# alibaba/unified-audio

Hardware: NVIDIA B200
Metric: hcodec2_encode_rvq_decode_samples_per_s (higher is better)
Workload: dtype f16x3/f16 tensor-core, f32 accumulate

## Files before the change

### unified_audio_b200/csrc/lstm_tc.cu

```cuda
#include <atomic>
#include <cstdio>
#include <cstdlib>

#include "common.cuh"
#include "quark_b200.h"

namespace qb {
extern std::atomic<long long> g_launches;

constexpr int LT_EPI_WARPS = 8, LT_THREADS = (LT_EPI_WARPS + 2) * 32;
constexpr int LT_KG = 4;
constexpr int LT_STAGES = 4;
constexpr uint32_t LT_KBLK = 32 * 128;
constexpr uint32_t LT_SLOT = LT_KBLK * LT_KG;
constexpr uint32_t LT_PAD = 12 * 1024;

__device__ __forceinline__ unsigned lt_ld_relaxed(const unsigned* p) {
  unsigned v;
  asm volatile("ld.relaxed.gpu.global.u32 %0, [%1];" : "=r"(v) : "l"(p) : "memory");
  return v;
}
__device__ __forceinline__ void bulk_load_1d(void* smem_dst, const void* gsrc, uint32_t bytes, uint64_t* bar) {
  asm volatile("cp.async.bulk.shared::cluster.global.mbarrier::complete_tx::bytes [%0], [%1], %2, [%3];"
               ::"r"(smem_u32(smem_dst)), "l"(gsrc), "r"(bytes), "r"(smem_u32(bar)) : "memory");
}
__device__ __forceinline__ void tmem_ld_32x32b_x8(uint32_t taddr, uint32_t (&r)[8]) {
  asm volatile("tcgen05.ld.sync.aligned.32x32b.x8.b32 {%0,%1,%2,%3,%4,%5,%6,%7}, [%8];"
               : "=r"(r[0]), "=r"(r[1]), "=r"(r[2]), "=r"(r[3]), "=r"(r[4]), "=r"(r[5]), "=r"(r[6]), "=r"(r[7])
               : "r"(taddr) : "memory");
}

__device__ __forceinline__ float lt_rcp(float x) {
  float r;
  asm("rcp.approx.ftz.f32 %0, %1;" : "=f"(r) : "f"(x));
  return r;
}
__device__ __forceinline__ float lt_sigmoid(float x) { return lt_rcp(1.0f + __expf(-x)); }
__device__ __forceinline__ float lt_tanh(float x) { return fmaf(-2.0f, lt_rcp(1.0f + __expf(2.0f * x)), 1.0f); }

__device__ __forceinline__ uint64_t lt_desc_core(uint32_t addr) {
  uint64_t d = 0;
  d |= (uint64_t)((addr & 0x3FFFF) >> 4);
  d |= (uint64_t)(128 >> 4) << 16;
  d |= (uint64_t)(128 >> 4) << 32;
  d |= (uint64_t)1 << 46;
  return d;
}
__device__ __forceinline__ void lt_cp_32x128b_warpx4(uint32_t taddr, uint64_t sdesc) {
  asm volatile("tcgen05.cp.cta_group::1.32x128b.warpx4 [%0], %1;" ::"r"(taddr), "l"(sdesc) : "memory");
}
__device__ __forceinline__ void lt_umma_ts(uint32_t tmem_d, uint32_t tmem_a, uint64_t desc_b, uint32_t idesc, uint32_t acc) {
  asm volatile(
      "{\n\t.reg .pred p;\n\t"
      "setp.ne.b32 p, %4, 0;\n\t"
      "tcgen05.mma.cta_group::1.kind::f16 [%0], [%1], %2, %3, p;\n\t}\n"
      ::"r"(tmem_d), "r"(tmem_a), "l"(desc_b), "r"(idesc), "r"(acc)
      : "memory");
}
constexpr uint32_t LT_TS_ACOL = 256;

template <int U, bool TS>
__global__ void __launch_bounds__(LT_THREADS, 1)
lstm_tc_kernel(const __grid_constant__ CUtensorMap tmW,
               const float* __restrict__ xp, int B, int T, int H, __half* __restrict__ out_hi,
               __half* __restrict__ out_lo, __half* hbuf, unsigned* flags, int Bp, int n_groups, int poll_ns, long long* prof) {
  constexpr int N = 4 * U;
  constexpr int HALF = U / 2;
  static_assert(N % 16 == 0 && N <= 64 && HALF * 4 % 8 == 0, "unsupported slice width");
  constexpr uint32_t WBLK = N * 128;
  constexpr uint32_t TCOLS = TS ? 512 : (4 * N <= 64 ? 64 : (4 * N <= 128 ? 128 : 256));
  extern __shared__ uint8_t smem_raw[];
  uint8_t* smem = (uint8_t*)(((uintptr_t)smem_raw + 1023) & ~(uintptr_t)1023);
  const int KB = H / 64;
  uint8_t* Wsm = smem;
  uint8_t* ring = smem + (size_t)KB * WBLK;
  uint64_t* full = (uint64_t*)(ring + LT_STAGES * LT_SLOT + LT_PAD);
  uint64_t* empty = full + LT_STAGES;
  uint64_t* wbar = empty + LT_STAGES;
  uint64_t* tfull = wbar + 1;
  uint32_t* tmem_slot = (uint32_t*)(tfull + 4);
  __shared__ long long ts_flag[4], ts_first[4], ts_last[4];

  const int tid = threadIdx.x, warp = tid >> 5, lane = tid & 31;
  const int u0 = blockIdx.x * U, G = gridDim.x;

  if (tid == 0) {
    for (int s = 0; s < LT_STAGES; ++s) { mbar_init(&full[s], 1); mbar_init(&empty[s], 1); }
    mbar_init(wbar, 1);
    for (int g = 0; g < 4; ++g) mbar_init(&tfull[g], 1);
    fence_mbar_init();
  }
  for (int i = tid; i < (int)((LT_STAGES * LT_SLOT + LT_PAD) / 16); i += LT_THREADS)
    reinterpret_cast<uint4*>(ring)[i] = make_uint4(0, 0, 0, 0);
  fence_proxy_async();
  if (warp == LT_EPI_WARPS + 1) { tmem_alloc(tmem_slot, TCOLS); tmem_relinquish(); }
  tc_fence_before();
  __syncthreads();
  tc_fence_after();
  const uint32_t tmem_base = *tmem_slot;

  if (warp == LT_EPI_WARPS) {
    if (lane == 0) {
      prefetch_tmap(&tmW);
      mbar_arrive_expect_tx(wbar, (uint32_t)KB * WBLK);
      for (int kb = 0; kb < KB; ++kb) tma_load_2d(Wsm + (size_t)kb * WBLK, &tmW, wbar, kb * 64, blockIdx.x * N);
    }
    uint32_t stage = 0, phase = 0;
    long long pw = 0;
    for (int t = 1; t < T; ++t) {
      for (int g = 0; g < n_groups; ++g) {
        const long long c0 = clock64();
        const unsigned* fl = flags + (size_t)g * G;
        unsigned spins = 0;
        for (;;) {
          bool ok = true;
          for (int c = lane; c < G; c += 32) ok = ok && (lt_ld_relaxed(fl + c) >= (unsigned)t);
          if (__all_sync(0xffffffffu, ok)) break;
          if (poll_ns) __nanosleep(poll_ns);
          if (++spins > (1u << 24)) asm volatile("trap;");
        }
        asm volatile("fence.acq_rel.gpu;" ::: "memory");
        __syncwarp();
        pw += clock64() - c0;
        if (lane == 0) {
          ts_flag[g] = clock64();
          asm volatile("fence.proxy.async;" ::: "memory");
          const int buf = (t + 1) & 1;
          for (int kb = 0; kb < KB; kb += LT_KG) {
            mbar_wait(&empty[stage], phase ^ 1);
            mbar_arrive_expect_tx(&full[stage], LT_SLOT);
            bulk_load_1d(ring + stage * LT_SLOT, hbuf + (((size_t)buf * n_groups + g) * KB + kb) * (LT_KBLK / 2), LT_SLOT,
                         &full[stage]);
            if (++stage == LT_STAGES) { stage = 0; phase ^= 1; }
          }
        }
        __syncwarp();
      }
    }
    if (prof && lane == 0 && blockIdx.x == 0) prof[0] = pw;
  } else if (warp == LT_EPI_WARPS + 1) {
    if (lane == 0) {
      constexpr uint32_t idesc = make_idesc_f16(128, N);
      mbar_wait(wbar, 0);
      uint32_t stage = 0, phase = 0, abuf = 0;
      for (int t = 1; t < T; ++t) {
        for (int g = 0; g < n_groups; ++g) {
          const uint32_t d_tmem = tmem_base + g * N;
          for (int kb0 = 0; kb0 < KB; kb0 += LT_KG) {
            mbar_wait(&full[stage], phase);
            tc_fence_after();
            if (kb0 == 0) ts_first[g] = clock64();
            if (TS) {
              const uint32_t a_tmem = tmem_base + LT_TS_ACOL + abuf * (LT_KG * 32);
              const uint32_t slot = smem_u32(ring + stage * LT_SLOT);
#pragma unroll
              for (int j = 0; j < LT_KG; ++j)
#pragma unroll
                for (int kc = 0; kc < 8; ++kc) lt_cp_32x128b_warpx4(a_tmem + j * 32 + kc * 4, lt_desc_core(slot + j * LT_KBLK + kc * 512));
#pragma unroll
              for (int j = 0; j < LT_KG; ++j) {
                const int kb = kb0 + j;
                const uint32_t sw = smem_u32(Wsm + (size_t)kb * WBLK);
#pragma unroll
                for (int k = 0; k < 4; ++k)
                  lt_umma_ts(d_tmem, a_tmem + j * 32 + k * 8, make_sw128_kmajor_desc(sw + k * 32), idesc, (kb | k) != 0 ? 1u : 0u);
              }
              abuf ^= 1;
            } else
#pragma unroll
            for (int j = 0; j < LT_KG; ++j) {
              const int kb = kb0 + j;
              const uint32_t sa = smem_u32(ring + stage * LT_SLOT + j * LT_KBLK) - (uint32_t)g * LT_KBLK;
              const uint32_t sw = smem_u32(Wsm + (size_t)kb * WBLK);
#pragma unroll
              for (int k = 0; k < 4; ++k)
                umma_f16(d_tmem, make_sw128_kmajor_desc(sa + k * 32), make_sw128_kmajor_desc(sw + k * 32), idesc,
                         (kb | k) != 0 ? 1u : 0u);
            }
            umma_commit(&empty[stage]);
            if (++stage == LT_STAGES) { stage = 0; phase ^= 1; }
          }
          umma_commit(&tfull[g]);
          ts_last[g] = clock64();
        }
      }
    }
  } else {
    const int g = warp & 3, half = warp >> 2;
    if (g < n_groups) {
      float c[HALF];
#pragma unroll
      for (int i = 0; i < HALF; ++i) c[i] = 0.f;
      const int n = g * 32 + lane;
      const bool act = n < B;
      const int u = u0 + half * HALF;
      long long ew = 0, ec = 0, ep = 0, pa = 0, pb = 0, pc = 0, pd = 0;
      for (int t = 0; t < T; ++t) {
        const long long e0 = clock64();
        __half* hcur = hbuf + ((size_t)(t & 1) * n_groups + g) * KB * (LT_KBLK / 2);
        float xg[4][HALF];
#pragma unroll
        for (int gg = 0; gg < 4; ++gg)
#pragma unroll
          for (int i = 0; i < HALF; ++i)
            xg[gg][i] = act ? xp[((long long)n * T + t) * 4 * H + (long long)gg * H + u + i] : 0.f;
        float acc[HALF * 4];
#pragma unroll
        for (int i = 0; i < HALF * 4; ++i) acc[i] = 0.f;
        long long e1 = e0;
        if (t > 0) {
          mbar_wait(&tfull[g], (t - 1) & 1);
          tc_fence_after();
          e1 = clock64();
          if (prof) {
            const volatile long long* vf = ts_flag; const volatile long long* v1 = ts_first; const volatile long long* v2 = ts_last;
            pa += vf[g] - e0; pb += v1[g] - vf[g]; pc += v2[g] - v1[g]; pd += e1 - v2[g];
          }
          const uint32_t taddr = tmem_base + ((uint32_t)(g * 32) << 16) + g * N + half * HALF * 4;
#pragma unroll
          for (int cc = 0; cc < HALF * 4; cc += 8) {
            uint32_t r[8];
            tmem_ld_32x32b_x8(taddr + cc, r);
            tmem_ld_wait();
#pragma unroll
            for (int e = 0; e < 8; ++e) acc[cc + e] = __uint_as_float(r[e]);
          }
        }
        if (act) {
          __half hv[HALF], lv[HALF];
#pragma unroll
          for (int i = 0; i < HALF; ++i) {
            const float gi = acc[4 * i] + xg[0][i], gf = acc[4 * i + 1] + xg[1][i];
            const float gc = acc[4 * i + 2] + xg[2][i], go = acc[4 * i + 3] + xg[3][i];
            const float ig = lt_sigmoid(gi), fg = lt_sigmoid(gf), cg = lt_tanh(gc), og = lt_sigmoid(go);
            const float cn = fg * c[i] + ig * cg;
            c[i] = cn;
            split_f16(og * lt_tanh(cn), hv[i], lv[i]);
          }
          const long long o = ((long long)n * T + t) * H + u;
#pragma unroll
          for (int i = 0; i < HALF; i += 2) {
            const __half2 h2 = __halves2half2(hv[i], hv[i + 1]);
            {
              const int uu = u + i, kbk = uu >> 6, col = uu & 63;
              const int off = TS ? kbk * (int)(LT_KBLK / 2) + ((((col >> 3) * 4 + (lane >> 3)) * 8 + (lane & 7)) << 3 | (col & 7))
                                 : kbk * (int)(LT_KBLK / 2) + lane * 64 + ((((col >> 3) ^ (lane & 7)) << 3) | (col & 7));
              *reinterpret_cast<__half2*>(hcur + off) = h2;
            }
            *reinterpret_cast<__half2*>(out_hi + o + i) = h2;
            if (out_lo) *reinterpret_cast<__half2*>(out_lo + o + i) = __halves2half2(lv[i], lv[i + 1]);
          }
        }
        tc_fence_before();
        asm volatile("bar.sync %0, 64;" ::"r"(1 + g) : "memory");
        const long long e2 = clock64();
        if (half == 0 && lane == 0) {
          asm volatile("st.release.gpu.global.u32 [%0], %1;" ::"l"(flags + (size_t)g * G + blockIdx.x), "r"((unsigned)(t + 1))
                       : "memory");
        }
        ew += e1 - e0; ec += e2 - e1; ep += clock64() - e2;
      }
      if (prof && warp == 0 && lane == 0 && blockIdx.x == 0) {
        prof[4] = ew; prof[5] = ec; prof[6] = ep; prof[1] = pa; prof[2] = pb; prof[3] = pc; prof[7] = pd;
      }
    }
  }
  tc_fence_before();
  __syncthreads();
  if (warp == LT_EPI_WARPS + 1) {
    __syncwarp();
    tc_fence_after();
    tmem_dealloc(tmem_base, TCOLS);
  }
}

typedef CUresult (*EncodeTiledFn)(CUtensorMap*, CUtensorMapDataType, cuuint32_t, void*, const cuuint64_t*,
                                  const cuuint64_t*, const cuuint32_t*, const cuuint32_t*, CUtensorMapInterleave,
                                  CUtensorMapSwizzle, CUtensorMapL2promotion, CUtensorMapFloatOOBfill);
static EncodeTiledFn lt_encode() {
  static EncodeTiledFn fn = nullptr;
  if (!fn) {
    void* p = nullptr;
    cudaDriverEntryPointQueryResult q;
    if (cudaGetDriverEntryPoint("cuTensorMapEncodeTiled", &p, cudaEnableDefault, &q) == cudaSuccess &&
        q == cudaDriverEntryPointSuccess)
      fn = (EncodeTiledFn)p;
  }
  return fn;
}

static int lstm_tc_chunk(const float* xp, const qb_half* whh_perm, int U, int B, int64_t T, int64_t H, __half* oh, __half* ol,
                         void* workspace, cudaStream_t st) {
  const int N = 4 * U, grid = (int)(H / U), KB = (int)(H / 64);
  const int n_groups = (B + 31) / 32, Bp = n_groups * 32;
  EncodeTiledFn enc = lt_encode();
  QB_REQUIRE(enc != nullptr, "cuTensorMapEncodeTiled not available");
  CUtensorMap tmW;
  {
    cuuint64_t dims[2] = {(cuuint64_t)H, (cuuint64_t)(4 * H)};
    cuuint64_t str[1] = {(cuuint64_t)H * 2};
    cuuint32_t box[2] = {64, (cuuint32_t)N};
    cuuint32_t es[2] = {1, 1};
    CUresult r = enc(&tmW, CU_TENSOR_MAP_DATA_TYPE_FLOAT16, 2, (void*)whh_perm, dims, str, box, es, CU_TENSOR_MAP_INTERLEAVE_NONE,
                     CU_TENSOR_MAP_SWIZZLE_128B, CU_TENSOR_MAP_L2_PROMOTION_L2_256B, CU_TENSOR_MAP_FLOAT_OOB_FILL_NONE);
    QB_REQUIRE(r == CUDA_SUCCESS, "lstm_tc: W tensor map failed (%d)", (int)r);
  }
  __half* hbuf = (__half*)workspace;
  const size_t smem = (size_t)KB * N * 128 + (size_t)LT_STAGES * LT_SLOT + LT_PAD + 1024 + 256;
  QB_REQUIRE(smem <= 227 * 1024, "lstm_tc: shared memory budget exceeded (%zu)", smem);
  const size_t hbytes = (size_t)2 * Bp * H * 2;
  QB_CHECK_CUDA(cudaMemsetAsync(workspace, 0, hbytes + 4096, st));
  unsigned* flags = (unsigned*)((uint8_t*)workspace + hbytes);
  static long long* prof = nullptr;
  if (!prof && getenv("QB_LSTM_PROF")) { cudaMalloc(&prof, 64); cudaMemset(prof, 0, 64); }
  int Bi = B, Ti = (int)T, Hi = (int)H, Bpi = Bp, ng = n_groups;
  static int poll_ns = -1;
  if (poll_ns < 0) { const char* e = getenv("QB_LSTM_POLL_NS"); poll_ns = e ? atoi(e) : 0; }
  void* args[] = {&tmW, &xp, &Bi, &Ti, &Hi, &oh, &ol, &hbuf, &flags, &Bpi, &ng, &poll_ns, &prof};
  static int ts_mode = -1;
  if (ts_mode < 0) { const char* e = getenv("QB_LSTM_TS"); ts_mode = e ? atoi(e) : 0; }
  const void* fn = ts_mode ? (U == 4 ? (const void*)lstm_tc_kernel<4, true> : U == 8 ? (const void*)lstm_tc_kernel<8, true>
                                                                                     : (const void*)lstm_tc_kernel<12, true>)
                           : (U == 4 ? (const void*)lstm_tc_kernel<4, false> : U == 8 ? (const void*)lstm_tc_kernel<8, false>
                                                                                      : (const void*)lstm_tc_kernel<12, false>);
  QB_CHECK_CUDA(cudaFuncSetAttribute(fn, cudaFuncAttributeMaxDynamicSharedMemorySize, (int)smem));
  QB_CHECK_CUDA(cudaLaunchCooperativeKernel(fn, dim3(grid), dim3(LT_THREADS), args, smem, st));
  g_launches++;
  if (prof) {
    long long h[8];
    cudaStreamSynchronize(st);
    cudaMemcpy(h, prof, 64, cudaMemcpyDeviceToHost);
    const double d = (double)Ti;
    fprintf(stderr, "[lstm_tc prof] cycles/step (cta0): producer flag-wait %.0f | epilogue(group0) wait-acc %.0f compute %.0f publish %.0f\n"
                    "               wait-acc split: step start -> all flags seen %.0f | -> first h stage landed %.0f | -> last MMA issued %.0f | -> accumulators ready %.0f\n",
            h[0] / d, h[4] / d, h[5] / d, h[6] / d, h[1] / d, h[2] / d, h[3] / d, h[7] / d);
  }
  return 0;
}

}
using namespace qb;

extern "C" int32_t qb_lstm_tc_units(int64_t H) {
  int dev = 0, sms = 0;
  if (cudaGetDevice(&dev) != cudaSuccess || cudaDeviceGetAttribute(&sms, cudaDevAttrMultiProcessorCount, dev) != cudaSuccess)
    sms = 148;
  for (int U : {4, 8, 12}) if (H % U == 0 && H / U <= sms) return U;
  return 0;
}

extern "C" int64_t qb_lstm_tc_workspace_bytes(int64_t B, int64_t H) {
  const int64_t Bc = B < 128 ? B : 128;
  const int64_t Bp = ceil_div(Bc, 32) * 32;
  return 2 * Bp * H * 2 + 4096;
}

extern "C" int qb_lstm_tc(const float* xp, const qb_half* whh_perm, int32_t units, int64_t B, int64_t T, int64_t H,
                          qb_half* out_hi, qb_half* out_lo, void* workspace, void* stream) {
  cudaStream_t st = (cudaStream_t)stream;
  QB_REQUIRE(xp && whh_perm && out_hi && workspace, "lstm_tc: bad args");
  QB_REQUIRE(H % (64 * LT_KG) == 0 && (units == 4 || units == 8 || units == 12) && H % units == 0, "lstm_tc: unsupported H / units");
  QB_REQUIRE(B >= 1, "lstm_tc: empty batch");
  for (int64_t b0 = 0; b0 < B; b0 += 128) {
    const int bc = (int)(B - b0 < 128 ? B - b0 : 128);
    if (int e = lstm_tc_chunk(xp + b0 * T * 4 * H, whh_perm, units, bc, T, H, (__half*)out_hi + b0 * T * H,
                              out_lo ? (__half*)out_lo + b0 * T * H : nullptr, workspace, st))
      return e;
  }
  return 0;
}
```

Measured before the change: 246.6 million.

## Restructure LSTM recurrence as 2-CTA cluster UMMA with weights as A operand

Rewrites the persistent LSTM tensor-core kernel so each pair of CTAs forms a cluster and issues cta_group::2 MMAs. The recurrent weights (64 gate rows per CTA) become the M operand and the hidden state the N operand, with each CTA loading half of the batch tile through a new TMA tensor map. The epilogue is reorganised around a shuffle-based gate transpose, and unit width is fixed at 16 so there are half as many CTAs. The aim is better MMA utilisation and less per-step synchronisation and load work, at the cost of cluster synchronisation, the removed TS mode and U options, and tighter H constraints.

Result: faster. 254.9 million, median of 6 (+3.3%).

```diff
diff --git a/unified_audio_b200/csrc/lstm_tc.cu b/unified_audio_b200/csrc/lstm_tc.cu
--- a/unified_audio_b200/csrc/lstm_tc.cu
+++ b/unified_audio_b200/csrc/lstm_tc.cu
@@ -8,25 +8,26 @@
 namespace qb {
 extern std::atomic<long long> g_launches;
 
+constexpr int LT_U = 16;
+constexpr int LT_ROWS = 4 * LT_U;
 constexpr int LT_EPI_WARPS = 8, LT_THREADS = (LT_EPI_WARPS + 2) * 32;
 constexpr int LT_KG = 4;
 constexpr int LT_STAGES = 4;
-constexpr uint32_t LT_KBLK = 32 * 128;
+constexpr uint32_t LT_KBLK = 16 * 128;
 constexpr uint32_t LT_SLOT = LT_KBLK * LT_KG;
-constexpr uint32_t LT_PAD = 12 * 1024;
+constexpr uint32_t LT_WBLK = LT_ROWS * 128;
+constexpr uint32_t LT_ACC_COLS = 32;
+constexpr uint32_t LT_TCOLS = 4 * LT_ACC_COLS;
 
 __device__ __forceinline__ unsigned lt_ld_relaxed(const unsigned* p) {
   unsigned v;
   asm volatile("ld.relaxed.gpu.global.u32 %0, [%1];" : "=r"(v) : "l"(p) : "memory");
   return v;
 }
-__device__ __forceinline__ void bulk_load_1d(void* smem_dst, const void* gsrc, uint32_t bytes, uint64_t* bar) {
-  asm volatile("cp.async.bulk.shared::cluster.global.mbarrier::complete_tx::bytes [%0], [%1], %2, [%3];"
-               ::"r"(smem_u32(smem_dst)), "l"(gsrc), "r"(bytes), "r"(smem_u32(bar)) : "memory");
-}
-__device__ __forceinline__ void tmem_ld_32x32b_x8(uint32_t taddr, uint32_t (&r)[8]) {
-  asm volatile("tcgen05.ld.sync.aligned.32x32b.x8.b32 {%0,%1,%2,%3,%4,%5,%6,%7}, [%8];"
-               : "=r"(r[0]), "=r"(r[1]), "=r"(r[2]), "=r"(r[3]), "=r"(r[4]), "=r"(r[5]), "=r"(r[6]), "=r"(r[7])
+__device__ __forceinline__ void tmem_ld_32x32b_x16(uint32_t taddr, uint32_t (&r)[16]) {
+  asm volatile("tcgen05.ld.sync.aligned.32x32b.x16.b32 {%0,%1,%2,%3,%4,%5,%6,%7,%8,%9,%10,%11,%12,%13,%14,%15}, [%16];"
+               : "=r"(r[0]), "=r"(r[1]), "=r"(r[2]), "=r"(r[3]), "=r"(r[4]), "=r"(r[5]), "=r"(r[6]), "=r"(r[7]), "=r"(r[8]),
+                 "=r"(r[9]), "=r"(r[10]), "=r"(r[11]), "=r"(r[12]), "=r"(r[13]), "=r"(r[14]), "=r"(r[15])
                : "r"(taddr) : "memory");
 }
 
@@ -38,43 +39,35 @@
 __device__ __forceinline__ float lt_sigmoid(float x) { return lt_rcp(1.0f + __expf(-x)); }
 __device__ __forceinline__ float lt_tanh(float x) { return fmaf(-2.0f, lt_rcp(1.0f + __expf(2.0f * x)), 1.0f); }
 
-__device__ __forceinline__ uint64_t lt_desc_core(uint32_t addr) {
-  uint64_t d = 0;
-  d |= (uint64_t)((addr & 0x3FFFF) >> 4);
-  d |= (uint64_t)(128 >> 4) << 16;
-  d |= (uint64_t)(128 >> 4) << 32;
-  d |= (uint64_t)1 << 46;
-  return d;
-}
-__device__ __forceinline__ void lt_cp_32x128b_warpx4(uint32_t taddr, uint64_t sdesc) {
-  asm volatile("tcgen05.cp.cta_group::1.32x128b.warpx4 [%0], %1;" ::"r"(taddr), "l"(sdesc) : "memory");
-}
-__device__ __forceinline__ void lt_umma_ts(uint32_t tmem_d, uint32_t tmem_a, uint64_t desc_b, uint32_t idesc, uint32_t acc) {
-  asm volatile(
-      "{\n\t.reg .pred p;\n\t"
-      "setp.ne.b32 p, %4, 0;\n\t"
-      "tcgen05.mma.cta_group::1.kind::f16 [%0], [%1], %2, %3, p;\n\t}\n"
-      ::"r"(tmem_d), "r"(tmem_a), "l"(desc_b), "r"(idesc), "r"(acc)
-      : "memory");
-}
-constexpr uint32_t LT_TS_ACOL = 256;
-
-template <int U, bool TS>
+__device__ __forceinline__ void lt_gate_transpose(float (&v)[16], int p) {
+#pragma unroll
+  for (int c = 0; c < 2; ++c)
+#pragma unroll
+    for (int i = 0; i < 4; ++i) {
+      const int a = 8 * c + i, b = 8 * c + 4 + i;
+      const float r = __shfl_xor_sync(0xffffffffu, (p & 1) ? v[a] : v[b], 1);
+      if (p & 1) v[a] = r; else v[b] = r;
+    }
+#pragma unroll
+  for (int c = 0; c < 2; ++c)
+#pragma unroll
+    for (int i = 0; i < 4; ++i) {
+      const int a = 4 * c + i, b = 4 * c + 8 + i;
+      const float r = __shfl_xor_sync(0xffffffffu, (p & 2) ? v[a] : v[b], 2);
+      if (p & 2) v[a] = r; else v[b] = r;
+    }
+}
+
 __global__ void __launch_bounds__(LT_THREADS, 1)
-lstm_tc_kernel(const __grid_constant__ CUtensorMap tmW,
+lstm_tc_kernel(const __grid_constant__ CUtensorMap tmW, const __grid_constant__ CUtensorMap tmH,
                const float* __restrict__ xp, int B, int T, int H, __half* __restrict__ out_hi,
-               __half* __restrict__ out_lo, __half* hbuf, unsigned* flags, int Bp, int n_groups, int poll_ns, long long* prof) {
-  constexpr int N = 4 * U;
-  constexpr int HALF = U / 2;
-  static_assert(N % 16 == 0 && N <= 64 && HALF * 4 % 8 == 0, "unsupported slice width");
-  constexpr uint32_t WBLK = N * 128;
-  constexpr uint32_t TCOLS = TS ? 512 : (4 * N <= 64 ? 64 : (4 * N <= 128 ? 128 : 256));
+               __half* __restrict__ out_lo, __half* hbuf, unsigned* flags, int n_groups, int poll_ns, long long* prof) {
   extern __shared__ uint8_t smem_raw[];
   uint8_t* smem = (uint8_t*)(((uintptr_t)smem_raw + 1023) & ~(uintptr_t)1023);
   const int KB = H / 64;
   uint8_t* Wsm = smem;
-  uint8_t* ring = smem + (size_t)KB * WBLK;
-  uint64_t* full = (uint64_t*)(ring + LT_STAGES * LT_SLOT + LT_PAD);
+  uint8_t* ring = smem + (size_t)KB * LT_WBLK;
+  uint64_t* full = (uint64_t*)(ring + LT_STAGES * LT_SLOT);
   uint64_t* empty = full + LT_STAGES;
   uint64_t* wbar = empty + LT_STAGES;
   uint64_t* tfull = wbar + 1;
@@ -82,7 +75,9 @@
   __shared__ long long ts_flag[4], ts_first[4], ts_last[4];
 
   const int tid = threadIdx.x, warp = tid >> 5, lane = tid & 31;
-  const int u0 = blockIdx.x * U, G = gridDim.x;
+  const int G = gridDim.x;
+  const uint32_t rank = cluster_ctarank();
+  const bool leader = rank == 0;
 
   if (tid == 0) {
     for (int s = 0; s < LT_STAGES; ++s) { mbar_init(&full[s], 1); mbar_init(&empty[s], 1); }
@@ -90,20 +85,19 @@
     for (int g = 0; g < 4; ++g) mbar_init(&tfull[g], 1);
     fence_mbar_init();
   }
-  for (int i = tid; i < (int)((LT_STAGES * LT_SLOT + LT_PAD) / 16); i += LT_THREADS)
-    reinterpret_cast<uint4*>(ring)[i] = make_uint4(0, 0, 0, 0);
-  fence_proxy_async();
-  if (warp == LT_EPI_WARPS + 1) { tmem_alloc(tmem_slot, TCOLS); tmem_relinquish(); }
+  if (warp == LT_EPI_WARPS + 1) { tmem_alloc2(tmem_slot, LT_TCOLS); tmem_relinquish2(); }
   tc_fence_before();
-  __syncthreads();
+  cluster_sync_all();
   tc_fence_after();
   const uint32_t tmem_base = *tmem_slot;
 
   if (warp == LT_EPI_WARPS) {
     if (lane == 0) {
       prefetch_tmap(&tmW);
-      mbar_arrive_expect_tx(wbar, (uint32_t)KB * WBLK);
-      for (int kb = 0; kb < KB; ++kb) tma_load_2d(Wsm + (size_t)kb * WBLK, &tmW, wbar, kb * 64, blockIdx.x * N);
+      prefetch_tmap(&tmH);
+      if (leader) mbar_arrive_expect_tx(wbar, 2u * KB * LT_WBLK);
+      const uint32_t wb = mapa_u32(smem_u32(wbar), 0);
+      for (int kb = 0; kb < KB; ++kb) tma2_load_2d(Wsm + (size_t)kb * LT_WBLK, &tmW, wb, kb * 64, blockIdx.x * LT_ROWS);
     }
     uint32_t stage = 0, phase = 0;
     long long pw = 0;
@@ -126,11 +120,11 @@
           ts_flag[g] = clock64();
           asm volatile("fence.proxy.async;" ::: "memory");
           const int buf = (t + 1) & 1;
+          const int row0 = (((buf * n_groups + g) * 2 + (int)rank) * KB) * 16;
           for (int kb = 0; kb < KB; kb += LT_KG) {
             mbar_wait(&empty[stage], phase ^ 1);
-            mbar_arrive_expect_tx(&full[stage], LT_SLOT);
-            bulk_load_1d(ring + stage * LT_SLOT, hbuf + (((size_t)buf * n_groups + g) * KB + kb) * (LT_KBLK / 2), LT_SLOT,
-                         &full[stage]);
+            if (leader) mbar_arrive_expect_tx(&full[stage], 2 * LT_SLOT);
+            tma2_load_2d(ring + stage * LT_SLOT, &tmH, mapa_u32(smem_u32(&full[stage]), 0), 0, row0 + kb * 16);
             if (++stage == LT_STAGES) { stage = 0; phase ^= 1; }
           }
         }
@@ -139,74 +133,61 @@
     }
     if (prof && lane == 0 && blockIdx.x == 0) prof[0] = pw;
   } else if (warp == LT_EPI_WARPS + 1) {
-    if (lane == 0) {
-      constexpr uint32_t idesc = make_idesc_f16(128, N);
+    if (lane == 0 && leader) {
+      constexpr uint32_t idesc = make_idesc_f16(128, 32);
       mbar_wait(wbar, 0);
-      uint32_t stage = 0, phase = 0, abuf = 0;
+      uint32_t stage = 0, phase = 0;
       for (int t = 1; t < T; ++t) {
         for (int g = 0; g < n_groups; ++g) {
-          const uint32_t d_tmem = tmem_base + g * N;
+          const uint32_t d_tmem = tmem_base + g * LT_ACC_COLS;
           for (int kb0 = 0; kb0 < KB; kb0 += LT_KG) {
             mbar_wait(&full[stage], phase);
             tc_fence_after();
             if (kb0 == 0) ts_first[g] = clock64();
-            if (TS) {
-              const uint32_t a_tmem = tmem_base + LT_TS_ACOL + abuf * (LT_KG * 32);
-              const uint32_t slot = smem_u32(ring + stage * LT_SLOT);
-#pragma unroll
-              for (int j = 0; j < LT_KG; ++j)
-#pragma unroll
-                for (int kc = 0; kc < 8; ++kc) lt_cp_32x128b_warpx4(a_tmem + j * 32 + kc * 4, lt_desc_core(slot + j * LT_KBLK + kc * 512));
-#pragma unroll
-              for (int j = 0; j < LT_KG; ++j) {
-                const int kb = kb0 + j;
-                const uint32_t sw = smem_u32(Wsm + (size_t)kb * WBLK);
-#pragma unroll
-                for (int k = 0; k < 4; ++k)
-                  lt_umma_ts(d_tmem, a_tmem + j * 32 + k * 8, make_sw128_kmajor_desc(sw + k * 32), idesc, (kb | k) != 0 ? 1u : 0u);
-              }
-              abuf ^= 1;
-            } else
 #pragma unroll
             for (int j = 0; j < LT_KG; ++j) {
-              const int kb = kb0 + j;
-              const uint32_t sa = smem_u32(ring + stage * LT_SLOT + j * LT_KBLK) - (uint32_t)g * LT_KBLK;
-              const uint32_t sw = smem_u32(Wsm + (size_t)kb * WBLK);
+              const uint32_t sw = smem_u32(Wsm + (size_t)(kb0 + j) * LT_WBLK);
+              const uint32_t sh = smem_u32(ring + stage * LT_SLOT + j * LT_KBLK);
 #pragma unroll
               for (int k = 0; k < 4; ++k)
-                umma_f16(d_tmem, make_sw128_kmajor_desc(sa + k * 32), make_sw128_kmajor_desc(sw + k * 32), idesc,
-                         (kb | k) != 0 ? 1u : 0u);
+                umma2_f16(d_tmem, make_sw128_kmajor_desc(sw + k * 32), make_sw128_kmajor_desc(sh + k * 32), idesc,
+                          ((kb0 + j) | k) != 0 ? 1u : 0u);
             }
-            umma_commit(&empty[stage]);
+            umma2_commit_mc(&empty[stage], 3);
             if (++stage == LT_STAGES) { stage = 0; phase ^= 1; }
           }
-          umma_commit(&tfull[g]);
+          umma2_commit_mc(&tfull[g], 3);
           ts_last[g] = clock64();
         }
       }
     }
   } else {
-    const int g = warp & 3, half = warp >> 2;
-    if (g < n_groups) {
-      float c[HALF];
-#pragma unroll
-      for (int i = 0; i < HALF; ++i) c[i] = 0.f;
-      const int n = g * 32 + lane;
-      const bool act = n < B;
-      const int u = u0 + half * HALF;
-      long long ew = 0, ec = 0, ep = 0, pa = 0, pb = 0, pc = 0, pd = 0;
-      for (int t = 0; t < T; ++t) {
+    const int q = warp & 3, s = warp >> 2, p = lane & 3;
+    const int unit = blockIdx.x * LT_U + 8 * (q & 1) + (lane >> 2);
+    const int bh = q >> 1;
+    const int kbk = unit >> 6, col = unit & 63;
+    float c[2][4];
+#pragma unroll
+    for (int gi = 0; gi < 2; ++gi)
+#pragma unroll
+      for (int i = 0; i < 4; ++i) c[gi][i] = 0.f;
+    long long ew = 0, ec = 0, ep = 0, pa = 0, pb = 0, pc = 0, pd = 0;
+    for (int t = 0; t < T; ++t) {
+#pragma unroll
+      for (int gi = 0; gi < 2; ++gi) {
+        const int g = s + 2 * gi;
+        if (g >= n_groups) break;
         const long long e0 = clock64();
-        __half* hcur = hbuf + ((size_t)(t & 1) * n_groups + g) * KB * (LT_KBLK / 2);
-        float xg[4][HALF];
+        const int n0 = g * 32 + bh * 16 + 4 * p;
+        float xg[4][4];
 #pragma unroll
         for (int gg = 0; gg < 4; ++gg)
 #pragma unroll
-          for (int i = 0; i < HALF; ++i)
-            xg[gg][i] = act ? xp[((long long)n * T + t) * 4 * H + (long long)gg * H + u + i] : 0.f;
-        float acc[HALF * 4];
-#pragma unroll
-        for (int i = 0; i < HALF * 4; ++i) acc[i] = 0.f;
+          for (int i = 0; i < 4; ++i)
+            xg[gg][i] = n0 + i < B ? xp[((long long)(n0 + i) * T + t) * 4 * H + (long long)gg * H + unit] : 0.f;
+        float v[16];
+#pragma unroll
+        for (int e = 0; e < 16; ++e) v[e] = 0.f;
         long long e1 = e0;
         if (t > 0) {
           mbar_wait(&tfull[g], (t - 1) & 1);
@@ -216,61 +197,52 @@
             const volatile long long* vf = ts_flag; const volatile long long* v1 = ts_first; const volatile long long* v2 = ts_last;
             pa += vf[g] - e0; pb += v1[g] - vf[g]; pc += v2[g] - v1[g]; pd += e1 - v2[g];
           }
-          const uint32_t taddr = tmem_base + ((uint32_t)(g * 32) << 16) + g * N + half * HALF * 4;
-#pragma unroll
-          for (int cc = 0; cc < HALF * 4; cc += 8) {
-            uint32_t r[8];
-            tmem_ld_32x32b_x8(taddr + cc, r);
-            tmem_ld_wait();
-#pragma unroll
-            for (int e = 0; e < 8; ++e) acc[cc + e] = __uint_as_float(r[e]);
+          uint32_t r[16];
+          tmem_ld_32x32b_x16(tmem_base + ((uint32_t)(q * 32) << 16) + g * LT_ACC_COLS, r);
+          tmem_ld_wait();
+#pragma unroll
+          for (int e = 0; e < 16; ++e) v[e] = __uint_as_float(r[e]);
+          lt_gate_transpose(v, p);
+        }
+        __half* hcur = hbuf + ((((size_t)(t & 1) * n_groups + g) * 2 + bh) * KB + kbk) * (LT_KBLK / 2);
+#pragma unroll
+        for (int i = 0; i < 4; ++i) {
+          const int n = n0 + i;
+          if (n < B) {
+            const float gi_ = v[i] + xg[0][i], gf = v[4 + i] + xg[1][i];
+            const float gc = v[8 + i] + xg[2][i], go = v[12 + i] + xg[3][i];
+            const float ig = lt_sigmoid(gi_), fg = lt_sigmoid(gf), cg = lt_tanh(gc), og = lt_sigmoid(go);
+            const float cn = fg * c[gi][i] + ig * cg;
+            c[gi][i] = cn;
+            __half hv, lv;
+            split_f16(og * lt_tanh(cn), hv, lv);
+            const int row = 4 * p + i;
+            hcur[row * 64 + ((((col >> 3) ^ (row & 7)) << 3) | (col & 7))] = hv;
+            const long long o = ((long long)n * T + t) * H + unit;
+            out_hi[o] = hv;
+            if (out_lo) out_lo[o] = lv;
           }
         }
-        if (act) {
-          __half hv[HALF], lv[HALF];
-#pragma unroll
-          for (int i = 0; i < HALF; ++i) {
-            const float gi = acc[4 * i] + xg[0][i], gf = acc[4 * i + 1] + xg[1][i];
-            const float gc = acc[4 * i + 2] + xg[2][i], go = acc[4 * i + 3] + xg[3][i];
-            const float ig = lt_sigmoid(gi), fg = lt_sigmoid(gf), cg = lt_tanh(gc), og = lt_sigmoid(go);
-            const float cn = fg * c[i] + ig * cg;
-            c[i] = cn;
-            split_f16(og * lt_tanh(cn), hv[i], lv[i]);
-          }
-          const long long o = ((long long)n * T + t) * H + u;
-#pragma unroll
-          for (int i = 0; i < HALF; i += 2) {
-            const __half2 h2 = __halves2half2(hv[i], hv[i + 1]);
-            {
-              const int uu = u + i, kbk = uu >> 6, col = uu & 63;
-              const int off = TS ? kbk * (int)(LT_KBLK / 2) + ((((col >> 3) * 4 + (lane >> 3)) * 8 + (lane & 7)) << 3 | (col & 7))
-                                 : kbk * (int)(LT_KBLK / 2) + lane * 64 + ((((col >> 3) ^ (lane & 7)) << 3) | (col & 7));
-              *reinterpret_cast<__half2*>(hcur + off) = h2;
-            }
-            *reinterpret_cast<__half2*>(out_hi + o + i) = h2;
-            if (out_lo) *reinterpret_cast<__half2*>(out_lo + o + i) = __halves2half2(lv[i], lv[i + 1]);
-          }
-        }
         tc_fence_before();
-        asm volatile("bar.sync %0, 64;" ::"r"(1 + g) : "memory");
+        asm volatile("bar.sync %0, 128;" ::"r"(1 + s) : "memory");
         const long long e2 = clock64();
-        if (half == 0 && lane == 0) {
+        if (q == 0 && lane == 0) {
           asm volatile("st.release.gpu.global.u32 [%0], %1;" ::"l"(flags + (size_t)g * G + blockIdx.x), "r"((unsigned)(t + 1))
                        : "memory");
         }
-        ew += e1 - e0; ec += e2 - e1; ep += clock64() - e2;
+        if (gi == 0) { ew += e1 - e0; ec += e2 - e1; ep += clock64() - e2; }
       }
-      if (prof && warp == 0 && lane == 0 && blockIdx.x == 0) {
-        prof[4] = ew; prof[5] = ec; prof[6] = ep; prof[1] = pa; prof[2] = pb; prof[3] = pc; prof[7] = pd;
-      }
+    }
+    if (prof && warp == 0 && lane == 0 && blockIdx.x == 0) {
+      prof[4] = ew; prof[5] = ec; prof[6] = ep; prof[1] = pa; prof[2] = pb; prof[3] = pc; prof[7] = pd;
     }
   }
   tc_fence_before();
-  __syncthreads();
+  cluster_sync_all();
   if (warp == LT_EPI_WARPS + 1) {
     __syncwarp();
     tc_fence_after();
-    tmem_dealloc(tmem_base, TCOLS);
+    tmem_dealloc2(tmem_base, LT_TCOLS);
   }
 }
 
@@ -289,42 +261,53 @@
   return fn;
 }
 
-static int lstm_tc_chunk(const float* xp, const qb_half* whh_perm, int U, int B, int64_t T, int64_t H, __half* oh, __half* ol,
+static int lstm_tc_chunk(const float* xp, const qb_half* whh_perm, int B, int64_t T, int64_t H, __half* oh, __half* ol,
                          void* workspace, cudaStream_t st) {
-  const int N = 4 * U, grid = (int)(H / U), KB = (int)(H / 64);
+  const int grid = (int)(H / LT_U), KB = (int)(H / 64);
   const int n_groups = (B + 31) / 32, Bp = n_groups * 32;
   EncodeTiledFn enc = lt_encode();
   QB_REQUIRE(enc != nullptr, "cuTensorMapEncodeTiled not available");
-  CUtensorMap tmW;
+  __half* hbuf = (__half*)workspace;
+  const size_t hbytes = (size_t)2 * Bp * H * 2;
+  CUtensorMap tmW, tmH;
   {
     cuuint64_t dims[2] = {(cuuint64_t)H, (cuuint64_t)(4 * H)};
     cuuint64_t str[1] = {(cuuint64_t)H * 2};
-    cuuint32_t box[2] = {64, (cuuint32_t)N};
+    cuuint32_t box[2] = {64, (cuuint32_t)LT_ROWS};
     cuuint32_t es[2] = {1, 1};
     CUresult r = enc(&tmW, CU_TENSOR_MAP_DATA_TYPE_FLOAT16, 2, (void*)whh_perm, dims, str, box, es, CU_TENSOR_MAP_INTERLEAVE_NONE,
                      CU_TENSOR_MAP_SWIZZLE_128B, CU_TENSOR_MAP_L2_PROMOTION_L2_256B, CU_TENSOR_MAP_FLOAT_OOB_FILL_NONE);
     QB_REQUIRE(r == CUDA_SUCCESS, "lstm_tc: W tensor map failed (%d)", (int)r);
   }
-  __half* hbuf = (__half*)workspace;
-  const size_t smem = (size_t)KB * N * 128 + (size_t)LT_STAGES * LT_SLOT + LT_PAD + 1024 + 256;
+  {
+    cuuint64_t dims[2] = {64, (cuuint64_t)(hbytes / 128)};
+    cuuint64_t str[1] = {128};
+    cuuint32_t box[2] = {64, 16 * LT_KG};
+    cuuint32_t es[2] = {1, 1};
+    CUresult r = enc(&tmH, CU_TENSOR_MAP_DATA_TYPE_FLOAT16, 2, (void*)hbuf, dims, str, box, es, CU_TENSOR_MAP_INTERLEAVE_NONE,
+                     CU_TENSOR_MAP_SWIZZLE_NONE, CU_TENSOR_MAP_L2_PROMOTION_L2_256B, CU_TENSOR_MAP_FLOAT_OOB_FILL_NONE);
+    QB_REQUIRE(r == CUDA_SUCCESS, "lstm_tc: h tensor map failed (%d)", (int)r);
+  }
+  const size_t smem = (size_t)KB * LT_WBLK + (size_t)LT_STAGES * LT_SLOT + 1024 + 256;
   QB_REQUIRE(smem <= 227 * 1024, "lstm_tc: shared memory budget exceeded (%zu)", smem);
-  const size_t hbytes = (size_t)2 * Bp * H * 2;
   QB_CHECK_CUDA(cudaMemsetAsync(workspace, 0, hbytes + 4096, st));
   unsigned* flags = (unsigned*)((uint8_t*)workspace + hbytes);
   static long long* prof = nullptr;
   if (!prof && getenv("QB_LSTM_PROF")) { cudaMalloc(&prof, 64); cudaMemset(prof, 0, 64); }
-  int Bi = B, Ti = (int)T, Hi = (int)H, Bpi = Bp, ng = n_groups;
+  int Bi = B, Ti = (int)T, Hi = (int)H, ng = n_groups;
   static int poll_ns = -1;
   if (poll_ns < 0) { const char* e = getenv("QB_LSTM_POLL_NS"); poll_ns = e ? atoi(e) : 0; }
-  void* args[] = {&tmW, &xp, &Bi, &Ti, &Hi, &oh, &ol, &hbuf, &flags, &Bpi, &ng, &poll_ns, &prof};
-  static int ts_mode = -1;
-  if (ts_mode < 0) { const char* e = getenv("QB_LSTM_TS"); ts_mode = e ? atoi(e) : 0; }
-  const void* fn = ts_mode ? (U == 4 ? (const void*)lstm_tc_kernel<4, true> : U == 8 ? (const void*)lstm_tc_kernel<8, true>
-                                                                                     : (const void*)lstm_tc_kernel<12, true>)
-                           : (U == 4 ? (const void*)lstm_tc_kernel<4, false> : U == 8 ? (const void*)lstm_tc_kernel<8, false>
-                                                                                      : (const void*)lstm_tc_kernel<12, false>);
+  void* args[] = {&tmW, &tmH, &xp, &Bi, &Ti, &Hi, &oh, &ol, &hbuf, &flags, &ng, &poll_ns, &prof};
+  const void* fn = (const void*)lstm_tc_kernel;
   QB_CHECK_CUDA(cudaFuncSetAttribute(fn, cudaFuncAttributeMaxDynamicSharedMemorySize, (int)smem));
-  QB_CHECK_CUDA(cudaLaunchCooperativeKernel(fn, dim3(grid), dim3(LT_THREADS), args, smem, st));
+  cudaLaunchConfig_t cfg = {};
+  cfg.gridDim = dim3(grid); cfg.blockDim = dim3(LT_THREADS); cfg.dynamicSmemBytes = smem; cfg.stream = st;
+  cudaLaunchAttribute at[2];
+  at[0].id = cudaLaunchAttributeCooperative; at[0].val.cooperative = 1;
+  at[1].id = cudaLaunchAttributeClusterDimension;
+  at[1].val.clusterDim.x = 2; at[1].val.clusterDim.y = 1; at[1].val.clusterDim.z = 1;
+  cfg.attrs = at; cfg.numAttrs = 2;
+  QB_CHECK_CUDA(cudaLaunchKernelExC(&cfg, fn, args));
   g_launches++;
   if (prof) {
     long long h[8];
@@ -345,8 +328,7 @@
   int dev = 0, sms = 0;
   if (cudaGetDevice(&dev) != cudaSuccess || cudaDeviceGetAttribute(&sms, cudaDevAttrMultiProcessorCount, dev) != cudaSuccess)
     sms = 148;
-  for (int U : {4, 8, 12}) if (H % U == 0 && H / U <= sms) return U;
-  return 0;
+  return (H % (2 * LT_U) == 0 && H % (64 * LT_KG) == 0 && H / LT_U <= sms) ? LT_U : 0;
 }
 
 extern "C" int64_t qb_lstm_tc_workspace_bytes(int64_t B, int64_t H) {
@@ -359,11 +341,11 @@
                           qb_half* out_hi, qb_half* out_lo, void* workspace, void* stream) {
   cudaStream_t st = (cudaStream_t)stream;
   QB_REQUIRE(xp && whh_perm && out_hi && workspace, "lstm_tc: bad args");
-  QB_REQUIRE(H % (64 * LT_KG) == 0 && (units == 4 || units == 8 || units == 12) && H % units == 0, "lstm_tc: unsupported H / units");
+  QB_REQUIRE(units == LT_U && H % (2 * LT_U) == 0 && H % (64 * LT_KG) == 0, "lstm_tc: unsupported H / units");
   QB_REQUIRE(B >= 1, "lstm_tc: empty batch");
   for (int64_t b0 = 0; b0 < B; b0 += 128) {
     const int bc = (int)(B - b0 < 128 ? B - b0 : 128);
-    if (int e = lstm_tc_chunk(xp + b0 * T * 4 * H, whh_perm, units, bc, T, H, (__half*)out_hi + b0 * T * H,
+    if (int e = lstm_tc_chunk(xp + b0 * T * 4 * H, whh_perm, bc, T, H, (__half*)out_hi + b0 * T * H,
                               out_lo ? (__half*)out_lo + b0 * T * H : nullptr, workspace, st))
       return e;
   }
```
